# tonymisic/audio-visual-tubes

Hardware: AMD Instinct MI355X
Metric: train-step clips/sec (whole node), ResNet18+VGG-M hard-way loss at 1/2/4/8 GPU (higher is better)
Workload: dtype bf16; 1 GPU; train_hardway_1frame step: 224x224 RGB + 257x300 spectrogram, fwd+CE+bwd+Adam; configs[1]; global_batch=128, per_gpu_batch=128, parallelism=dp1

## Files before the change

audio-visual-tubes_amd/_lib.py:

```python
from __future__ import annotations

import ctypes
import os
import subprocess
import threading

PKG_DIR = os.path.dirname(os.path.abspath(__file__))
CSRC = os.path.join(PKG_DIR, "csrc")
LIB_PATH = os.path.join(PKG_DIR, "libavt.so")
LOAD_PATH = os.environ.get("AVT_LIB_PATH", LIB_PATH)
SOURCES = ["conv_gemm.hip", "bn.hip", "pool.hip", "head.hip", "misc.hip", "tube.hip", "conv3d_bwd.hip", "eval.hip", "audio.hip", "frames.hip"]

_P = ctypes.c_void_p
_I = ctypes.c_int
_L = ctypes.c_longlong
_F = ctypes.c_float
_Z = ctypes.c_size_t

class DgradBnEpi(ctypes.Structure):
    _fields_ = [("xc", ctypes.c_void_p), ("y", ctypes.c_void_p), ("stats", ctypes.c_void_p),
                ("acc", ctypes.c_void_p), ("xc2", ctypes.c_void_p), ("stats2", ctypes.c_void_p),
                ("acc2", ctypes.c_void_p), ("skip_class00", ctypes.c_int), ("append_slots", ctypes.c_int)]


# ... 27 lines not shown
    "avt_set_halo_stages": (_I, [_I, _I]),
    "avt_set_c64": (_I, [_I]),
    "avt_set_s2_dgrad_one": (_I, [_I]),
    "avt_set_stem_kernel": (_I, [_I]),
    "avt_set_stem_wgrad": (_I, [_I]),
    "avt_set_nt128_config": (_I, [_I]),
    "avt_set_wgrad_slab_max": (_I, [_I, _I]),
    "avt_set_wgrad_tiles": (_I, [_I]),
    "avt_set_small_tiles": (_I, [_I]),
    "avt_set_wgrad_halo": (_I, [_I]),
    "avt_set_wgrad_row3": (_I, [_I, _I, _I]),
    "avt_set_halo3d": (_I, [_I]),
    "avt_set_halo_tps2": (_I, [_I]),
    "avt_set_wgrad_fused": (_I, [_I, _I]),
    "avt_conv2d_wgrad_tickets": (_I, [_I, _I, _I, _I, _I, _I, _I, _I, _I, _I]),
    "avt_conv2d_wgrad_tk": (_I, [_P, _P, _P, _I, _I, _I, _I, _I, _I, _I, _I, _I, _I, _P, _Z, _P, _I, _P]),
    "avt_conv2d_wgrad_defer": (_I, [_P, _P, _P, _I, _I, _I, _I, _I, _I, _I, _I, _I, _I, _P, _Z,
                                    ctypes.POINTER(SlabReduceDesc), _P]),
    "avt_wgrad_reduce_batch": (_I, [ctypes.POINTER(SlabReduceDesc), _I, _P]),
    "avt_bn_acc_doubles": (_Z, [_L, _I]),
    "avt_conv2d_fwd": (_I, [_P, _P, _P, _P, _I, _I, _I, _I, _I, _I, _I, _I, _I, _I, _P]),
    "avt_conv2d_dgrad": (_I, [_P, _P, _P, _P, _I, _I, _I, _I, _I, _I, _I, _I, _I, _P]),
    "avt_conv2d_dgrad_bn": (_I, [_P, _P, _P, _P, _I, _I, _I, _I, _I, _I, _I, _I, _I, ctypes.POINTER(DgradBnEpi), _P]),
    "avt_bn_bwd_premasked": (_I, [_P, _P, _P, _P, _P, _P, _P, _P, _P, _L, _I, _P]),
    "avt_conv2d_dgrad_mask": (_I, [_P, _P, _P, _P, _P, _I, _I, _I, _I, _I, _I, _I, _I, _I, _P]),
    "avt_conv2d_splitk_plan": (_I, [_I, _I, _I, _I, _I, _I, _I, _I, _I, _I, _P, _P]),
    "avt_set_halo_splitk": (_I, [_I, _I]),
    "avt_set_wgrad_nst": (_I, [_I, _I]),
    "avt_set_wgrad_slots_pct": (_I, [_I]),
    "avt_conv2d_fwd_ws": (_I, [_P, _P, _P, _P, _I, _I, _I, _I, _I, _I, _I, _I, _I, _I, _P, _L, _P, _I, _P]),
    "avt_conv2d_dgrad_ws": (_I, [_P, _P, _P, _P, _P, _I, _I, _I, _I, _I, _I, _I, _I, _I, _P, _L, _P, _I, _P]),
    "avt_bn_apply_mask": (_I, [_P, _P, _P, _P, _P, _P, _P, _P, _L, _I, _P]),
    "avt_bn_bwd_mask": (_I, [_P, _P, ctypes.POINTER(BnBwdTarget), ctypes.POINTER(BnBwdTarget), _L, _I, _P]),
    "avt_conv2d_wgrad_workspace": (_Z, [_I, _I, _I, _I, _I, _I, _I, _I, _I, _I]),
    "avt_conv2d_wgrad": (_I, [_P, _P, _P, _I, _I, _I, _I, _I, _I, _I, _I, _I, _I, _P, _Z, _P]),
    "avt_bn_finalize": (_I, [_P, _L, _I, _P, _P, _P, _P, _F, _F, _P, _P, _P, _P, _P]),
    "avt_bn_finalize_rep": (_I, [_P, _L, _L, _I, _P, _P, _P, _P, _F, _F, _P, _P, _P, _P, _P]),
    "avt_conv3d_fwd": (_I, [_P, _P, _P, _P, _I, _I, _I, _I, _I, _I, _I, _I, _I, _I, _I, _I, _P]),
    "avt_video_stem_im2col": (_I, [_P, _P, _I, _I, _I, _I, _I, _I, _I, _P]),
    "avt_maxpool3d_fwd": (_I, [_P, _P, _I, _I, _I, _I, _I, _P]),
    "avt_pack_conv3d_weight_dgrad": (_I, [_P, _P, _I, _I, _I, _I, _I, _P]),
    "avt_pack_conv3d_weights_dgrad_batched": (_I, [_P, _I, _I, _P]),
    "avt_conv3d_dgrad": (_I, [_P, _P, _P, _P, _I, _I, _I, _I, _I, _I, _I, _I, _I, _I, _I, _I, _P]),
    "avt_conv3d_wgrad_workspace": (_Z, [_I, _I, _I, _I, _I, _I, _I, _I, _I, _I, _I, _I]),
    "avt_conv3d_wgrad": (_I, [_P, _P, _P, _I, _I, _I, _I, _I, _I, _I, _I, _I, _I, _I, _I, _P, _Z, _P]),
    "avt_maxpool3d_bwd": (_I, [_P, _P, _P, _P, _I, _I, _I, _I, _I, _P]),
# ... 152 lines not shown
```

audio-visual-tubes_amd/csrc/conv_epi.h:

```cpp
#pragma once

__device__ __forceinline__ u32x4 epi_mask8(u32x4 v, unsigned bits) {
  unsigned* u = reinterpret_cast<unsigned*>(&v);
#pragma unroll
  for (int e = 0; e < 4; ++e)
    u[e] &= ((bits >> (2 * e)) & 1u ? 0x0000ffffu : 0u) | ((bits >> (2 * e + 1)) & 1u ? 0xffff0000u : 0u);
  return v;
}

__device__ __forceinline__ void epi_unpack8(const u32x4& v, float* f) {
  const unsigned* u = reinterpret_cast<const unsigned*>(&v);
#pragma unroll
  for (int e = 0; e < 4; ++e) {
    f[2 * e] = bf2f(u[e] & 0xffff);
    f[2 * e + 1] = bf2f(u[e] >> 16);
  }
}

template <int NT, int BM, int BN, int UMAX, typename OrowFn>
__device__ __forceinline__ void epi_store_bn(const GemmNTParams& p, const bf16_t* Ct, int ct_ld, int n0, int rows_valid,
                                             int mt, int nrow_tiles, OrowFn orow, float* scratch) {
  constexpr int OCPR = BN / 8;
  static_assert(NT % OCPR == 0 && 64 % OCPR == 0, "a thread keeps one channel chunk");
  const int tid = threadIdx.x;
  const bool bnb = p.bx != nullptr;
  const bool two = p.bx2 != nullptr;
  const int cc = tid % OCPR;
  const int c0 = n0 + cc * 8;
  float s1[8], s2[8], s3[8];
#pragma unroll
  for (int e = 0; e < 8; ++e) s1[e] = s2[e] = s3[e] = 0.f;
  constexpr int ITERS = BM * OCPR / NT;
  static_assert(ITERS * NT == BM * OCPR, "rows per thread");
  constexpr int U = ITERS < UMAX ? ITERS : UMAX;
  const bool has_add = p.add != nullptr, has_y = p.by != nullptr;
  for (int it0 = 0; it0 < ITERS; it0 += U) {
    u32x4 aa[U], xx[U], yy[U], x2[U];
    size_t off[U];
// ... 45 lines not shown
          for (int e = 0; e < 8; ++e)
            g[e] = __builtin_fmaf(xc[e], bst[c0 + e], bst[p.Ng + c0 + e]) > 0.f ? g[e] : 0.f;
        }
#pragma unroll
        for (int e = 0; e < 8; ++e) {
          s1[e] += g[e];
          s2[e] += g[e] * ((xc[e] - bst[2 * p.Ng + c0 + e]) * bst[3 * p.Ng + c0 + e]);
        }
        if (two) {
          float xb[8];
          epi_unpack8(x2[u], xb);
#pragma unroll
          for (int e = 0; e < 8; ++e)
            s3[e] += g[e] * ((xb[e] - bst2[2 * p.Ng + c0 + e]) * bst2[3 * p.Ng + c0 + e]);
        }
        unsigned* vp = reinterpret_cast<unsigned*>(&v);
#pragma unroll
        for (int e = 0; e < 4; ++e) vp[e] = pack2(g[2 * e], g[2 * e + 1]);
      }
      *reinterpret_cast<u32x4*>(p.out + off[u]) = v;
    }
  }
  if (!bnb) return;
#pragma unroll
  for (int m = OCPR; m < 64; m <<= 1)
#pragma unroll
    for (int e = 0; e < 8; ++e) {
      s1[e] += __shfl_xor(s1[e], m, 64);
      s2[e] += __shfl_xor(s2[e], m, 64);
      if (two) s3[e] += __shfl_xor(s3[e], m, 64);
    }
  constexpr int NW = NT / 64;
  const int lane = tid & 63, wid = tid >> 6;
  __syncthreads();
  if (lane < OCPR) {
#pragma unroll
    for (int e = 0; e < 8; ++e) {
      float* q = scratch + ((size_t)wid * BN + cc * 8 + e) * 3;
      q[0] = s1[e];
      q[1] = s2[e];
      q[2] = s3[e];
    }
  }
  __syncthreads();
  const int total = p.bslot_total ? p.bslot_total : nrow_tiles;
  bn_write_header(p.bacc, total, p.bappend);
  if (two) bn_write_header(p.bacc2, total, p.bappend);
  const size_t slot = (size_t)(p.bslot_base + bn_slot_base(p.bacc, p.bappend) + mt);
  const size_t slot2 = two ? (size_t)(p.bslot_base + bn_slot_base(p.bacc2, p.bappend) + mt) : 0;
  for (int c = tid; c < BN; c += NT) {
    float a = 0.f, b = 0.f, d = 0.f;
#pragma unroll
    for (int w = 0; w < NW; ++w) {
      const float* q = scratch + ((size_t)w * BN + c) * 3;
      a += q[0];
      b += q[1];
      d += q[2];
    }
    double* acc = bn_bwd_slots(p.bacc, p.Ng) + (slot * p.Ng + n0 + c) * 2;
    acc[0] = (double)a;
    acc[1] = (double)b;
    if (two) {
      double* acc2 = bn_bwd_slots(p.bacc2, p.Ng) + (slot2 * p.Ng + n0 + c) * 2;
      acc2[0] = (double)a;
      acc2[1] = (double)d;
    }
  }
}

template <int NT, int BM, int BN, bool EPI, typename OrowFn, int UMAX = 4>
__device__ __forceinline__ void epi_store(const GemmNTParams& p, const bf16_t* Ct, int ct_ld, int n0, int rows_valid,
                                          int mt, int nrow_tiles, OrowFn orow, float* scratch) {
  if constexpr (!EPI) {
    constexpr int OCPR = BN / 8;
    for (int idx = threadIdx.x; idx < BM * OCPR; idx += NT) {
      const int r = idx / OCPR, cc = idx - r * OCPR;
      if (r >= rows_valid) continue;
      u32x4 v = *reinterpret_cast<const u32x4*>(Ct + r * ct_ld + cc * 8);
      const size_t off = orow(r) * (size_t)p.Ng + n0 + cc * 8;
      if (p.add != nullptr) {
        u32x4 a = *reinterpret_cast<const u32x4*>(p.add + off);
        if (p.amask != nullptr) a = epi_mask8(a, p.amask[off >> 3]);
        unsigned* vv = reinterpret_cast<unsigned*>(&v);
        const unsigned* aa = reinterpret_cast<const unsigned*>(&a);
#pragma unroll
        for (int e = 0; e < 4; ++e) {
          const float lo = bf2f(vv[e] & 0xffff) + bf2f(aa[e] & 0xffff);
          const float hi = bf2f(vv[e] >> 16) + bf2f(aa[e] >> 16);
          vv[e] = pack2(lo, hi);
        }
      }
      *reinterpret_cast<u32x4*>(p.out + off) = v;
    }
    return;
  } else {
    epi_store_bn<NT, BM, BN, UMAX>(p, Ct, ct_ld, n0, rows_valid, mt, nrow_tiles, orow, scratch);
  }
}
```

audio-visual-tubes_amd/csrc/conv_gemm.hip:

```cpp
#include "avt_common.h"

namespace avt {

#include "conv_params.h"

template <int MODE, int CVEC, int BM, int BN>
__global__ __launch_bounds__(256) void gemm_nt_kernel(GemmNTParams p) {
  constexpr int TM = BM / 64, TN = BN / 64;
  constexpr int AR = BM / 64, BR = BN / 64;
  constexpr int STAGE_BYTES = 2 * (BM + BN) * 64;
  constexpr int CT_LD = BN + 8;
  constexpr int EPI_BYTES = BM * CT_LD * 2;
  constexpr int SMEM = (STAGE_BYTES > EPI_BYTES ? STAGE_BYTES : EPI_BYTES);
  __shared__ __attribute__((aligned(16))) char smem[SMEM + 4 * BN * 4];
  float* red = reinterpret_cast<float*>(smem + SMEM);

  const int tid = threadIdx.x, lane = tid & 63, wid = tid >> 6;
  const int wm = wid >> 1, wn = wid & 1;
  const int nnt = p.Ng / BN;
  const int mt = blockIdx.x / nnt, nt = blockIdx.x % nnt;
  const int m0 = mt * BM, n0 = nt * BN;

  const int lchunk = tid & 3, lrow = tid >> 2;
  int a_pix[AR], a_y[AR], a_x[AR];
// ... 733 lines not shown
static bool halo_eligible(const GemmNTParams& p) {
  const int h = halo_enabled();
  if (!h || p.R != 3 || p.S != 3 || p.stride != 1 || p.pad != 1 || p.IC % 64 != 0 || p.IT > 1 || p.OT > 1 || p.KT > 1 ||
      p.IH != p.OH || p.IW != p.OW)
    return false;
  if (h == 2) return 256 + 2 * p.OW + 2 <= kHaloPR && (p.Ng % 128 == 0 || p.Ng == 64);
  static const int l2 = getenv("AVT_HALO_L2") ? atoi(getenv("AVT_HALO_L2")) : 1;
  return p.Ng % 128 == 0 && (128 + 2 * p.OW + 2 <= 168 || (l2 && 256 + 2 * p.OW + 2 <= kHaloPR));
}

static bool use_small_tile(const GemmNTParams& p, int BN) {
  if (g_small_tile_pct == -2) {
    const char* e = getenv("AVT_SMALL_TILES");
    const char* ep = getenv("AVT_SMALL_TILES_PCT");
    const int w = e ? atoi(e) : 1;
    g_small_tile_pct = e ? (w > 0 ? 100 * w : w) : ep ? atoi(ep) : 50;
  }
  if (g_small_tile_pct == 0) return false;
  if (g_small_tile_pct < 0) return true;
  const long long blocks128 = (long long)((p.M + 127) / 128) * (p.Ng / BN);
  return blocks128 * 100 < (long long)g_small_tile_pct * num_cus();
}

template <int MODE, int WM, int WN, int TM, int TN, int NSTB, int PRMAX, bool EPI, int OPT = 0>
static void launch_halo_one(const GemmNTParams& p, const HaloArgs& ha, int grid, hipStream_t st) {
  hipLaunchKernelGGL((conv_halo_kernel<MODE, WM, WN, TM, TN, NSTB, PRMAX, EPI, false, 0, OPT>), dim3(grid),
                     dim3(WM * WN * 64), 0, st, p, ha);
}

template <int MODE, int WM, int WN, int TM, int TN, int NSTB = 3, int PRMAX = kHaloPR, int OPT = 0>
static void launch_halo(const GemmNTParams& p, hipStream_t st, int ksplit = 1, float* part = nullptr,
                        int* cnt = nullptr) {
  constexpr int BM = WM * TM * 32, BN = WN * TN * 32;
  HaloArgs ha{};
  ha.ksplit = ksplit;
  ha.cps = p.IC / 64 / ksplit;
#ifdef AVT_DIAG
  static const int hdbg = getenv("AVT_HALO_DBG") ? atoi(getenv("AVT_HALO_DBG")) : 0;
  ha.dbg = hdbg;
#endif
  ha.part = part;
  ha.cnt = cnt;
  const int batch = p.M / (p.OH * p.OW);
  ha.act_bytes = (unsigned)((size_t)batch * p.IH * p.IW * p.IC * 2);
  ha.w_bytes = (unsigned)((size_t)p.Ng * p.Kg * 2);
  ha.W = p.OW;
  ha.H = p.OH;
  for (int r = 0; r < 3; ++r)
    for (int s = 0; s < 3; ++s) {
      const int t = r * 3 + s;
      const int dy = MODE == MODE_FWD ? r - 1 : 1 - r, dx = MODE == MODE_FWD ? s - 1 : 1 - s;
      ha.tap_dy[t] = dy;
      ha.tap_dx[t] = dx;
      ha.tap_disp[t] = dy * p.OW + dx;
      ha.tap_w[t] = t;
    }
  if constexpr ((OPT & 4) != 0) {
    ha.T = p.IT;
    ha.div_hw = make_magic((unsigned)(p.OH * p.OW));
    ha.div_t = make_magic((unsigned)p.IT);
  }
  const int grid = ((p.M + BM - 1) / BM) * (p.Ng / BN) * ksplit;
  if (grid > 0 && ksplit > 1) {
    hipLaunchKernelGGL((conv_halo_kernel<MODE, WM, WN, TM, TN, NSTB, PRMAX, false, true>), dim3(grid),
                       dim3(WM * WN * 64), 0, st, p, ha);
    return;
  }
  if (grid <= 0) return;
  if constexpr ((OPT & 4) != 0)
    launch_halo_one<MODE, WM, WN, TM, TN, NSTB, PRMAX, false, OPT>(p, ha, grid, st);
  else if (MODE == MODE_DGRAD && p.bx != nullptr)
    launch_halo_one<MODE, WM, WN, TM, TN, NSTB, PRMAX, true, OPT>(p, ha, grid, st);
  else
    launch_halo_one<MODE, WM, WN, TM, TN, NSTB, PRMAX, false, OPT>(p, ha, grid, st);
}

static int g_halo_tps2 = -1;
static int halo_tps2(const GemmNTParams& p, int vt = 1) {
  if (g_halo_tps2 < 0) g_halo_tps2 = getenv("AVT_HALO_TPS2") ? atoi(getenv("AVT_HALO_TPS2")) : 0;
  const int nv = p.IC / 64 * vt;
  return g_halo_tps2 && p.IC % 64 == 0 && nv % 2 == 0 && nv >= 8;
}

static int g_halo3d = -1;
static int halo3d_enabled() {
  if (g_halo3d < 0) g_halo3d = getenv("AVT_HALO3D") ? atoi(getenv("AVT_HALO3D")) : 2;
  return g_halo3d;
}
static bool halo3d_launch(const GemmNTParams& p, hipStream_t st) {
  if (!halo3d_enabled() || p.KT != 3 || p.R != 3 || p.S != 3 || p.stride != 1 || p.pad != 1 || p.pad_t != 1 ||
      p.IT != p.OT || p.IH != p.OH || p.IW != p.OW || p.IC % 64 != 0 || conv_variant() != 1)
    return false;
  if (p.Ng == 64) {
    if (halo3d_enabled() < 2 || 256 + 2 * p.OW + 2 > 488) return false;
    launch_halo<MODE_FWD, 8, 1, 1, 2, 3, 488, 4>(p, st);
    return true;
  }
// ... 364 lines not shown
  if (C % 128 == 0)
    launch_nt<MODE_DGRAD, 8, 128, 128>(p, st, ws);
  else
    launch_nt<MODE_DGRAD, 8, 128, 64>(p, st);
  return check_launch("conv2d_dgrad");
}

extern "C" int avt_conv2d_dgrad_ws(const void* dy, const void* wt, void* dx, const void* add, const void* add_mask,
                                   int N, int H, int W, int C, int K, int R, int S, int stride, int pad, float* part,
                                   long long part_floats, int* cnt, int counters, void* stream) {
  AVT_REQUIRE(add_mask == nullptr || (add && add != dx), "conv2d_dgrad_ws: add_mask needs add, not aliasing dx");
  AVT_REQUIRE(part_floats >= 0 && counters >= 0, "conv2d_dgrad_ws: negative workspace size");
  const SplitWs ws{part, cnt, part_floats, counters};
  return conv2d_dgrad_impl(dy, wt, dx, add, add_mask, N, H, W, C, K, R, S, stride, pad, nullptr, stream,
                           (part && cnt) ? &ws : nullptr);
}

extern "C" int avt_conv2d_dgrad_bn(const void* dy, const void* wt, void* dx, const void* add, int N, int H, int W,
                                   int C, int K, int R, int S, int stride, int pad, const avt_dgrad_bn_epi* epi,
                                   void* stream) {
  return conv2d_dgrad_impl(dy, wt, dx, add, nullptr, N, H, W, C, K, R, S, stride, pad, epi, stream);
}

extern "C" int avt_conv2d_dgrad(const void* dy, const void* wt, void* dx, const void* add, int N, int H, int W, int C,
                                int K, int R, int S, int stride, int pad, void* stream) {
  return conv2d_dgrad_impl(dy, wt, dx, add, nullptr, N, H, W, C, K, R, S, stride, pad, nullptr, stream);
}

extern "C" int avt_conv2d_dgrad_mask(const void* dy, const void* wt, void* dx, const void* add, const void* add_mask,
                                     int N, int H, int W, int C, int K, int R, int S, int stride, int pad,
                                     void* stream) {
  AVT_REQUIRE(add && add_mask, "conv2d_dgrad_mask: add and add_mask are required");
  AVT_REQUIRE(add != dx, "conv2d_dgrad_mask: add must not alias dx");
  return conv2d_dgrad_impl(dy, wt, dx, add, add_mask, N, H, W, C, K, R, S, stride, pad, nullptr, stream);
}

static int conv3d_fwd_impl(const void* x, const void* wpack, void* y, double* bn_acc, const void* add, int N, int T,
                           int H, int W, int Cp, int K, int KT, int R, int S, int stride, int pad_t, int pad,
                           void* stream) {
  AVT_REQUIRE(x && wpack && y, "conv3d_fwd: null pointer");
  AVT_REQUIRE(K % 64 == 0, "conv3d_fwd: K=%d must be a multiple of 64", K);
  AVT_REQUIRE(Cp % 32 == 0, "conv3d_fwd: C=%d must be a multiple of 32", Cp);
  AVT_REQUIRE(KT * R * S <= kMaxTaps && KT >= 1 && R >= 1 && S >= 1, "conv3d_fwd: at most %d taps", kMaxTaps);
  AVT_REQUIRE(stride == 1 || stride == 2, "conv3d_fwd: spatial stride must be 1 or 2");
  GemmNTParams p{};
  p.act = (const bf16_t*)x;
// ... 692 lines not shown
```

audio-visual-tubes_amd/csrc/conv_halo.h:

```cpp
#pragma once

struct HaloArgs {
  unsigned act_bytes, w_bytes;
  int W, H;
  int tap_disp[9];
  int tap_dy[9], tap_dx[9];
  int tap_w[9];
  int ksplit, cps;
  float* part;
  int* cnt;
  int dbg;
  int T;
  MagicDiv div_hw, div_t;
};
#ifdef AVT_DIAG
#define HALO_DBG(bit) (ha.dbg & (bit))
#else
#define HALO_DBG(bit) false
#endif


__device__ __forceinline__ int halo_swz(int row) { return (row >> 1) & 7; }

template <int WN, int TN, int NSTB, int PRMAX, int TPS = 1>
constexpr int halo_blocks_per_cu() {
  return 2 * (2 * (PRMAX * 128 + 1024) + NSTB * TPS * WN * TN * 32 * 128 + 4096) <= 160 * 1024 ? 2 : 1;
}

template <int MODE, int WM, int WN, int TM, int TN, int NSTB, int PRMAX, bool EPI = false, bool SPLIT = false,
          int PREF = 0, int OPT = 0>
__global__ __launch_bounds__(WM * WN * 64, (halo_blocks_per_cu<WN, TN, NSTB, PRMAX, (OPT & 2) ? 2 : 1>())) void conv_halo_kernel(
    GemmNTParams p, HaloArgs ha) {
  constexpr int FR = 32, FM = TM, FN = TN;
  constexpr int KD = 16;
  constexpr int NW = WM * WN, NT = NW * 64;
  constexpr int BM = WM * TM * 32, BN = WN * TN * 32;
  constexpr int BK = 64, RB = 128, RPI = 8;
  constexpr int BR = BN / (NW * RPI);
  static_assert(BR >= 1 && BR * NW * RPI == BN, "weight tile / wave split");
  constexpr int PINSTR = (PRMAX + RPI - 1) / RPI;
  static_assert(NSTB >= 2 && NSTB <= 5, "NSTB");
  constexpr int NPIECE = 10 - NSTB;
  constexpr int AP = (PINSTR + NPIECE * NW - 1) / (NPIECE * NW);
  constexpr int ABUF = PRMAX * RB + 1024;
  constexpr int BSTAGE = BN * RB;
  constexpr int TPS = (OPT & 2) ? 2 : 1;
  constexpr int CT_LD = BN + 8;
  constexpr int EPI_BYTES = BM * CT_LD * 2;
  constexpr int MAIN = 2 * ABUF + NSTB * TPS * BSTAGE;
  constexpr int SMEM = (MAIN > EPI_BYTES ? MAIN : EPI_BYTES);
  static_assert(PRMAX % RPI == 0, "PRMAX");
  static_assert(SMEM + 2 * WM * BN * 4 <= 160 * 1024, "LDS budget of a CU");
// ... 411 lines not shown
          if (acc_row(i, v) < rows_valid) q += d * d;
        }
#pragma unroll
      for (int o = FR; o < 64; o <<= 1) q += __shfl_xor(q, o, 64);
      if (lane < FR) red[WM * BN + wm * BN + cc] = q;
    }
    __syncthreads();
    bn_write_header(p.stats, (p.M + BM - 1) / BM, 0, mt == 0 && n0 == 0);
    double* acc_slot = bn_fwd_slots(p.stats) + (size_t)mt * p.Ng * 3;
    for (int cc = tid; cc < BN; cc += NT) {
      double sd = 0.0, m2 = 0.0;
#pragma unroll
      for (int k = 0; k < WM; ++k) {
        sd += (double)red[k * BN + cc];
        m2 += (double)red[WM * BN + k * BN + cc];
      }
      double* a = acc_slot + (size_t)(n0 + cc) * 3;
      a[0] = sd;
      a[1] = m2;
      a[2] = sd * sd / (double)rows_valid;
    }
  }
  bf16_t* Ct = reinterpret_cast<bf16_t*>(smem);
#pragma unroll
  for (int i = 0; i < FM; ++i)
#pragma unroll
    for (int j = 0; j < FN; ++j)
#pragma unroll
      for (int v = 0; v < AV; ++v) Ct[acc_row(i, v) * CT_LD + wn * (BN / WN) + j * FR + frow] = f2bf(acc[i][j][v]);
  __syncthreads();
  if (!HALO_DBG(16))
    epi_store<NT, BM, BN, EPI>(p, Ct, CT_LD, n0, rows_valid, mt, (p.M + BM - 1) / BM,
                               [&](int r) -> size_t { return (size_t)(m0 + r); },
                        reinterpret_cast<float*>(smem));
}
```

audio-visual-tubes_amd/trunk.py:

```python
from __future__ import annotations

import ctypes
import os
from dataclasses import dataclass
from typing import Dict, List, Optional

import torch

from ._lib import BnBwdTarget, DgradBnEpi, SlabReduceDesc, call, query

STAGES = [(64, 1), (128, 2), (256, 2), (512, 1)]
FUSE_BN_BWD = os.environ.get("AVT_FUSE_BN_BWD", "0") == "1"
DIAG_H1_SKIP = os.environ.get("AVT_DIAG_H1_SKIP", "0") == "1"
if DIAG_H1_SKIP and os.environ.get("AVT_DIAG_WRONG_RESULTS_OK", "0") != "1":
    raise RuntimeError("avt: AVT_DIAG_H1_SKIP=1 computes WRONG results (timing diagnostic); set "
                       "AVT_DIAG_WRONG_RESULTS_OK=1 as well to run it (tools/step_time.py)")


def P(t: Optional[torch.Tensor]):
    return None if t is None else ctypes.c_void_p(t.data_ptr())


def stream_ptr():
    return ctypes.c_void_p(torch.cuda.current_stream().cuda_stream)


def drive(gen):
    while True:
        try:
            next(gen)
        except StopIteration as e:
            return e.value


def conv_out(n: int, k: int, s: int, p: int) -> int:
# ... 304 lines not shown
                pending.append((d, ws))
        else:
            call("avt_conv2d_wgrad_tk", P(x), P(gy), P(dw), N, H, W, spec.cp, spec.cin, spec.cout, spec.k, spec.k,
                 spec.stride, spec.pad, P(ws), wsb, P(tk), 0 if tk is None else tk.numel(), stream_ptr())
        ConvProfiler.end(ev, "wgrad", 2.0 * gy.numel() * spec.k * spec.k * spec.cin,
                         2.0 * (x.numel() + gy.numel()) + 8.0 * dw.numel())

    def flush_wgrad(self, store: Store):
        pending = store.wgrad_pending(self.prefix)
        if not pending:
            return
        arr = (SlabReduceDesc * len(pending))(*[d for d, _ in pending])
        call("avt_wgrad_reduce_batch", arr, len(pending), stream_ptr())
        pending.clear()

    def _dgrad(self, gy, N, H, W, spec: ConvSpec, store: Store, add=None, inplace=False, epi=None, add_mask=None):
        _, wt = store.packed(spec)
        gx = add if inplace else torch.empty(N, H, W, spec.cin, device=gy.device, dtype=torch.bfloat16)
        ws = store.splitk(spec, True, N, H, W) if epi is None else None
        ev = ConvProfiler.begin()
        if ws is not None:
            call("avt_conv2d_dgrad_ws", P(gy), P(wt), P(gx), P(add), P(add_mask), N, H, W, spec.cin, spec.cout,
                 spec.k, spec.k, spec.stride, spec.pad, P(ws[0]), ws[0].numel(), P(ws[1]), ws[1].numel(), stream_ptr())
        elif add_mask is not None:
            assert epi is None
            call("avt_conv2d_dgrad_mask", P(gy), P(wt), P(gx), P(add), P(add_mask), N, H, W, spec.cin, spec.cout,
                 spec.k, spec.k, spec.stride, spec.pad, stream_ptr())
        elif epi is None:
            call("avt_conv2d_dgrad", P(gy), P(wt), P(gx), P(add), N, H, W, spec.cin, spec.cout, spec.k, spec.k,
                 spec.stride, spec.pad, stream_ptr())
        else:
            call("avt_conv2d_dgrad_bn", P(gy), P(wt), P(gx), P(add), N, H, W, spec.cin, spec.cout, spec.k, spec.k,
                 spec.stride, spec.pad, ctypes.byref(epi), stream_ptr())
        ConvProfiler.end(ev, "dgrad", 2.0 * gy.numel() * spec.k * spec.k * spec.cin,
                         2.0 * (gy.numel() + wt.numel() + gx.numel() * (2 if add is not None else 1)))
        return gx

    HI_BLOCK = 4

    def backward(self, tape: Dict, g_out: torch.Tensor, store: Store, on_boundary=None):
        g, pm = self.backward_blocks(tape, g_out, store, self.HI_BLOCK, len(self.blocks))
        if on_boundary is not None:
            on_boundary(self.prefix + "hi")
        g, _ = self.backward_blocks(tape, g, store, 0, self.HI_BLOCK, pm)
        self.backward_stem(tape, g, store)

    def _bn_bwd_premasked(self, gm, xc, stats, bn: BNSpec, store: Store):
        gc = torch.empty_like(xc)
        call("avt_bn_bwd_premasked", P(gm), P(xc), P(stats[2]), P(stats[3]), P(store.param(bn.prefix + ".weight")),
             P(store.grad(bn.prefix + ".weight")), P(store.grad(bn.prefix + ".bias")), P(gc),
             P(store.stat_acc(bn, "bwd", xc.numel() // bn.c)), xc.numel() // bn.c, bn.c, stream_ptr())
        return gc

    def _epi(self, store: Store, bn: BNSpec, xc, stats, y=None, bn2: Optional[BNSpec] = None, xc2=None, stats2=None,
             skip00: bool = False, append: bool = False) -> DgradBnEpi:
        e = DgradBnEpi()
        rows = xc.numel() // bn.c
        e.xc, e.y, e.stats = xc.data_ptr(), (y.data_ptr() if y is not None else None), stats.data_ptr()
        e.acc = store.stat_acc(bn, "bwd", rows).data_ptr()
        if bn2 is not None:
            e.xc2, e.stats2, e.acc2 = xc2.data_ptr(), stats2.data_ptr(), store.stat_acc(bn2, "bwd", rows).data_ptr()
        e.skip_class00 = int(skip00)
        e.append_slots = int(append)
        return e

    def backward_blocks(self, tape: Dict, g: torch.Tensor, store: Store, lo: int, hi: int, premasked: bool = False):
        return drive(self.backward_blocks_iter(tape, g, store, lo, hi, premasked))

    def backward_blocks_iter(self, tape: Dict, g: torch.Tensor, store: Store, lo: int, hi: int,
                             premasked: bool = False):
        N = tape["N"]
        ev = not tape.get("training", True)
        pgrad = not (ev and tape.get("frozen", False))
        fuse = FUSE_BN_BWD and not ev
        for bi in reversed(range(lo, hi)):
            blk, t = self.blocks[bi], tape["blocks"][bi]
            Hc, Wc, Ho, Wo = t["H"], t["W"], t["Ho"], t["Wo"]
            identity = blk["down"] is None
            if premasked:
                gres = g
                g_c2 = self._bn_bwd_premasked(g, t["c2"], t["s2"], blk["bn2"], store)
                g_cd = None if identity else self._bn_bwd_premasked(g, t["cd"], t["sd"], blk["bnd"], store)
            else:
                gres = None
                if ev:
                    g_c2, g_cd = self._bn_eval_bwd_mask(g, t["om"], t["c2"], t["s2"], blk["bn2"], store, pgrad,
                                                        *(() if identity else (t["cd"], t["sd"], blk["bnd"])))
                elif identity and fuse and bi > 0:
                    gres = torch.empty_like(t["c2"])
                    g_c2 = self._bn_bwd(g, t["out"], t["c2"], t["s2"], blk["bn2"], store, gmask_out=gres)
                    g_cd = None
                elif identity:
                    g_c2, g_cd = self._bn_bwd_mask(g, t["om"], t["c2"], t["s2"], blk["bn2"], store)
                else:
                    g_c2, g_cd = self._bn_bwd_mask(g, t["om"], t["c2"], t["s2"], blk["bn2"], store,
                                                   t["cd"], t["sd"], blk["bnd"])
            yield
            if pgrad:
                self._wgrad(t["h1"], g_c2, N, Ho, Wo, blk["conv2"], store)
            yield
            if fuse:
                g_h1 = self._dgrad(g_c2, N, Ho, Wo, blk["conv2"], store,
                                   epi=self._epi(store, blk["bn1"], t["c1"], t["s1"]))
                g_c1 = self._bn_bwd_premasked(g_h1, t["c1"], t["s1"], blk["bn1"], store)
            else:
                g_h1 = self._dgrad(g_c2, N, Ho, Wo, blk["conv2"], store)
                yield
                if ev:
                    g_c1 = self._bn_eval_relu_bwd(g_h1, t["c1"], t["s1"], blk["bn1"], store, pgrad)
                else:
                    g_c1 = self._bn_relu_bwd(g_h1, t["c1"], t["s1"], blk["bn1"], store)
            yield
            if pgrad:
                self._wgrad(t["x"], g_c1, N, Hc, Wc, blk["conv1"], store)
                yield
                if not identity:
                    self._wgrad(t["x"], g_cd, N, Hc, Wc, blk["down"], store)
                    yield
            epi = None
            if bi > 0 and fuse:
                pb, pt = self.blocks[bi - 1], tape["blocks"][bi - 1]
                has_d = pb["down"] is not None
                mk = lambda skip00, append=False: self._epi(
                    store, pb["bn2"], pt["c2"], pt["s2"], y=pt["out"], bn2=pb["bnd"] if has_d else None,
                    xc2=pt["cd"] if has_d else None, stats2=pt["sd"] if has_d else None, skip00=skip00, append=append)
                epi = mk(False)
            if identity and gres is None:
                g_x = self._dgrad(g_c1, N, Hc, Wc, blk["conv1"], store, add=g, epi=epi, add_mask=t["om"])
            elif identity:
                g_x = self._dgrad(g_c1, N, Hc, Wc, blk["conv1"], store, add=gres, epi=epi)
            else:
                strided = blk["conv1"].stride == 2
                g_x = self._dgrad(g_c1, N, Hc, Wc, blk["conv1"], store,
                                  epi=mk(True) if (epi is not None and strided) else None)
                if epi is not None and strided:
                    epi = mk(False, append=True)
                g_x = self._dgrad(g_cd, N, Hc, Wc, blk["down"], store, add=g_x, inplace=True, epi=epi)
            g = g_x
            premasked = epi is not None
            yield
        return g, premasked

    def backward_stem(self, tape: Dict, g: torch.Tensor, store: Store):
# ... 38 lines not shown
```

include/avt.h:

```cpp
#ifndef AVT_H_
#define AVT_H_

#include <stddef.h>

#ifdef __cplusplus
extern "C" {
#endif

#define AVT_OK 0
#define AVT_EINVAL -1
#define AVT_EHIP -2

const char* avt_last_error(void);
int avt_abi_version(void);
#define AVT_BUILD_DIAG 1
int avt_build_flags(void);

int avt_peak_mfma(float* sink, int shape, int blocks, int iters, unsigned seed, void* stream);
long long avt_peak_mfma_flops(int shape, int blocks, int iters);
int avt_copy16(void* dst, const void* src, size_t bytes, int blocks, void* stream);

size_t avt_bn_acc_doubles(long long rows, int C);
int avt_conv2d_fwd(const void* x, const void* wpack, void* y, double* bn_acc, int N, int H, int W, int Cp, int K,
                   int R, int S, int stride, int pad, int Kg, void* stream);
// ... 2 lines not shown
int avt_conv2d_dgrad_mask(const void* dy, const void* wt, void* dx, const void* add, const void* add_mask, int N,
                          int H, int W, int C, int K, int R, int S, int stride, int pad, void* stream);
int avt_conv2d_splitk_plan(int N, int H, int W, int C, int K, int R, int S, int stride, int pad, int dgrad,
                           long long* part_floats, int* counters);
int avt_conv2d_fwd_ws(const void* x, const void* wpack, void* y, double* bn_acc, int N, int H, int W, int Cp, int K,
                      int R, int S, int stride, int pad, int Kg, float* part, long long part_floats, int* cnt,
                      int counters, void* stream);
int avt_conv2d_dgrad_ws(const void* dy, const void* wt, void* dx, const void* add, const void* add_mask, int N,
                        int H, int W, int C, int K, int R, int S, int stride, int pad, float* part,
                        long long part_floats, int* cnt, int counters, void* stream);
typedef struct {
  const void* xc;
  const void* y;
  const float* stats;
  double* acc;
  const void* xc2;
  const float* stats2;
  double* acc2;
  int skip_class00;
  int append_slots;
} avt_dgrad_bn_epi;
int avt_conv2d_dgrad_bn(const void* dy, const void* wt, void* dx, const void* add, int N, int H, int W, int C, int K,
                        int R, int S, int stride, int pad, const avt_dgrad_bn_epi* epi, void* stream);
size_t avt_conv2d_wgrad_workspace(int N, int H, int W, int Cp, int Creal, int K, int R, int S, int stride, int pad);
int avt_conv2d_wgrad(const void* x, const void* dy, float* dw, int N, int H, int W, int Cp, int Creal, int K, int R,
                     int S, int stride, int pad, void* workspace, size_t ws_bytes, void* stream);
typedef struct {
  const float* slab;
  float* dw;
  int splits, tiles, nnt, Mg, ldw;
  int wm, wn, tm, tn;
} avt_slab_reduce_desc;
int avt_conv2d_wgrad_defer(const void* x, const void* dy, float* dw, int N, int H, int W, int Cp, int Creal, int K,
                           int R, int S, int stride, int pad, void* workspace, size_t ws_bytes, avt_slab_reduce_desc* desc,
                           void* stream);
int avt_wgrad_reduce_batch(const avt_slab_reduce_desc* descs, int n, void* stream);
int avt_conv2d_wgrad_tickets(int N, int H, int W, int Cp, int Creal, int K, int R, int S, int stride, int pad);
int avt_conv2d_wgrad_tk(const void* x, const void* dy, float* dw, int N, int H, int W, int Cp, int Creal, int K, int R,
                        int S, int stride, int pad, void* workspace, size_t ws_bytes, int* tickets, int n_tickets,
                        void* stream);

int avt_conv_stem_dgrad(const void* gy, const float* w, float* gx, int N, int H, int W, int Cin, void* stream);

int avt_conv3d_fwd(const void* x, const void* wpack, void* y, double* bn_acc, int N, int T, int H, int W, int Cp,
                   int K, int KT, int R, int S, int stride, int pad_t, int pad, void* stream);
int avt_video_stem_im2col(const float* x, void* out, int N, int C, int T, int H, int W, int KT, int pad_t,
// ... 140 lines not shown
```

Before: 13060 clips/s.

## Enable fused BN-backward dgrad epilogue by default with per-shape planning

Turns BN-backward fusion into the dgrad halo kernel on by default, but only for conv2 shapes where a planner confirms the halo path is used without split-K. Adds a restructured halo epilogue that prefetches the BN inputs and per-channel constants into registers and LDS before the accumulator store, plus a specialised variant without residual or mask operands. Also adds a masked-add dgrad+BN entry point. This removes separate BN-backward reduction passes and their memory traffic, at the cost of more register and LDS pressure in the epilogue, and relies on the planner's heuristic choice of shapes.

```diff
diff --git a/audio-visual-tubes_amd/_lib.py b/audio-visual-tubes_amd/_lib.py
--- a/audio-visual-tubes_amd/_lib.py
+++ b/audio-visual-tubes_amd/_lib.py
@@ -73,6 +73,9 @@
     "avt_conv2d_fwd": (_I, [_P, _P, _P, _P, _I, _I, _I, _I, _I, _I, _I, _I, _I, _I, _P]),
     "avt_conv2d_dgrad": (_I, [_P, _P, _P, _P, _I, _I, _I, _I, _I, _I, _I, _I, _I, _P]),
     "avt_conv2d_dgrad_bn": (_I, [_P, _P, _P, _P, _I, _I, _I, _I, _I, _I, _I, _I, _I, ctypes.POINTER(DgradBnEpi), _P]),
+    "avt_conv2d_dgrad_bn_mask": (_I, [_P, _P, _P, _P, _P, _I, _I, _I, _I, _I, _I, _I, _I, _I,
+                                      ctypes.POINTER(DgradBnEpi), _P]),
+    "avt_conv2d_dgrad_bn_plan": (_I, [_I, _I, _I, _I, _I, _I, _I, _I, _I, _P]),
     "avt_bn_bwd_premasked": (_I, [_P, _P, _P, _P, _P, _P, _P, _P, _P, _L, _I, _P]),
     "avt_conv2d_dgrad_mask": (_I, [_P, _P, _P, _P, _P, _I, _I, _I, _I, _I, _I, _I, _I, _I, _P]),
     "avt_conv2d_splitk_plan": (_I, [_I, _I, _I, _I, _I, _I, _I, _I, _I, _I, _P, _P]),
diff --git a/audio-visual-tubes_amd/csrc/conv_epi.h b/audio-visual-tubes_amd/csrc/conv_epi.h
--- a/audio-visual-tubes_amd/csrc/conv_epi.h
+++ b/audio-visual-tubes_amd/csrc/conv_epi.h
@@ -14,6 +14,59 @@
   for (int e = 0; e < 4; ++e) {
     f[2 * e] = bf2f(u[e] & 0xffff);
     f[2 * e + 1] = bf2f(u[e] >> 16);
+  }
+}
+
+template <int NT, int BN>
+__device__ __forceinline__ void epi_bn_tail(const GemmNTParams& p, float* s1, float* s2, float* s3, int n0, int mt,
+                                            int nrow_tiles, float* scratch) {
+  constexpr int OCPR = BN / 8;
+  const int tid = threadIdx.x;
+  const bool two = p.bx2 != nullptr;
+  const int cc = tid % OCPR;
+#pragma unroll
+  for (int m = OCPR; m < 64; m <<= 1)
+#pragma unroll
+    for (int e = 0; e < 8; ++e) {
+      s1[e] += __shfl_xor(s1[e], m, 64);
+      s2[e] += __shfl_xor(s2[e], m, 64);
+      if (two) s3[e] += __shfl_xor(s3[e], m, 64);
+    }
+  constexpr int NW = NT / 64;
+  const int lane = tid & 63, wid = tid >> 6;
+  __syncthreads();
+  if (lane < OCPR) {
+#pragma unroll
+    for (int e = 0; e < 8; ++e) {
+      float* q = scratch + ((size_t)wid * BN + cc * 8 + e) * 3;
+      q[0] = s1[e];
+      q[1] = s2[e];
+      q[2] = s3[e];
+    }
+  }
+  __syncthreads();
+  const int total = p.bslot_total ? p.bslot_total : nrow_tiles;
+  bn_write_header(p.bacc, total, p.bappend);
+  if (two) bn_write_header(p.bacc2, total, p.bappend);
+  const size_t slot = (size_t)(p.bslot_base + bn_slot_base(p.bacc, p.bappend) + mt);
+  const size_t slot2 = two ? (size_t)(p.bslot_base + bn_slot_base(p.bacc2, p.bappend) + mt) : 0;
+  for (int c = tid; c < BN; c += NT) {
+    float a = 0.f, b = 0.f, d = 0.f;
+#pragma unroll
+    for (int w = 0; w < NW; ++w) {
+      const float* q = scratch + ((size_t)w * BN + c) * 3;
+      a += q[0];
+      b += q[1];
+      d += q[2];
+    }
+    double* acc = bn_bwd_slots(p.bacc, p.Ng) + (slot * p.Ng + n0 + c) * 2;
+    acc[0] = (double)a;
+    acc[1] = (double)b;
+    if (two) {
+      double* acc2 = bn_bwd_slots(p.bacc2, p.Ng) + (slot2 * p.Ng + n0 + c) * 2;
+      acc2[0] = (double)a;
+      acc2[1] = (double)d;
+    }
   }
 }
 
@@ -105,50 +158,7 @@
     }
   }
   if (!bnb) return;
-#pragma unroll
-  for (int m = OCPR; m < 64; m <<= 1)
-#pragma unroll
-    for (int e = 0; e < 8; ++e) {
-      s1[e] += __shfl_xor(s1[e], m, 64);
-      s2[e] += __shfl_xor(s2[e], m, 64);
-      if (two) s3[e] += __shfl_xor(s3[e], m, 64);
-    }
-  constexpr int NW = NT / 64;
-  const int lane = tid & 63, wid = tid >> 6;
-  __syncthreads();
-  if (lane < OCPR) {
-#pragma unroll
-    for (int e = 0; e < 8; ++e) {
-      float* q = scratch + ((size_t)wid * BN + cc * 8 + e) * 3;
-      q[0] = s1[e];
-      q[1] = s2[e];
-      q[2] = s3[e];
-    }
-  }
-  __syncthreads();
-  const int total = p.bslot_total ? p.bslot_total : nrow_tiles;
-  bn_write_header(p.bacc, total, p.bappend);
-  if (two) bn_write_header(p.bacc2, total, p.bappend);
-  const size_t slot = (size_t)(p.bslot_base + bn_slot_base(p.bacc, p.bappend) + mt);
-  const size_t slot2 = two ? (size_t)(p.bslot_base + bn_slot_base(p.bacc2, p.bappend) + mt) : 0;
-  for (int c = tid; c < BN; c += NT) {
-    float a = 0.f, b = 0.f, d = 0.f;
-#pragma unroll
-    for (int w = 0; w < NW; ++w) {
-      const float* q = scratch + ((size_t)w * BN + c) * 3;
-      a += q[0];
-      b += q[1];
-      d += q[2];
-    }
-    double* acc = bn_bwd_slots(p.bacc, p.Ng) + (slot * p.Ng + n0 + c) * 2;
-    acc[0] = (double)a;
-    acc[1] = (double)b;
-    if (two) {
-      double* acc2 = bn_bwd_slots(p.bacc2, p.Ng) + (slot2 * p.Ng + n0 + c) * 2;
-      acc2[0] = (double)a;
-      acc2[1] = (double)d;
-    }
-  }
+  epi_bn_tail<NT, BN>(p, s1, s2, s3, n0, mt, nrow_tiles, scratch);
 }
 
 template <int NT, int BM, int BN, bool EPI, typename OrowFn, int UMAX = 4>
@@ -180,3 +190,115 @@
     epi_store_bn<NT, BM, BN, UMAX>(p, Ct, ct_ld, n0, rows_valid, mt, nrow_tiles, orow, scratch);
   }
 }
+
+template <int NT, int BM, int BN, bool GEN>
+struct EpiBnHalo {
+  static constexpr int OCPR = BN / 8;
+  static constexpr int ITERS = BM * OCPR / NT;
+  static constexpr int CST_FLOATS = 6 * BN;
+  static_assert(NT % OCPR == 0 && 64 % OCPR == 0 && ITERS * NT == BM * OCPR && NT >= BN, "rows per thread");
+  u32x4 xx[ITERS];
+  u32x4 aa[GEN ? ITERS : 1], yy[GEN ? ITERS : 1], x2[GEN ? ITERS : 1];
+  unsigned am[GEN ? ITERS : 1];
+  float kc[6];
+
+  __device__ __forceinline__ void load(const GemmNTParams& p, int n0, size_t m0, int rows_valid) {
+    const int tid = threadIdx.x;
+    const int c0 = n0 + (tid % OCPR) * 8;
+    if (tid < BN) {
+#pragma unroll
+      for (int k = 0; k < 4; ++k) kc[k] = p.bst[k * p.Ng + n0 + tid];
+      if (GEN && p.bx2 != nullptr) {
+        kc[4] = p.bst2[2 * p.Ng + n0 + tid];
+        kc[5] = p.bst2[3 * p.Ng + n0 + tid];
+      }
+    }
+#pragma unroll
+    for (int u = 0; u < ITERS; ++u) {
+      const int r = (tid + u * NT) / OCPR;
+      if (r >= rows_valid) continue;
+      const size_t off = (m0 + r) * (size_t)p.Ng + c0;
+      xx[u] = *reinterpret_cast<const u32x4*>(p.bx + off);
+      if constexpr (GEN) {
+        if (p.by != nullptr) yy[u] = *reinterpret_cast<const u32x4*>(p.by + off);
+        if (p.bx2 != nullptr) x2[u] = *reinterpret_cast<const u32x4*>(p.bx2 + off);
+        if (p.add != nullptr) {
+          aa[u] = *reinterpret_cast<const u32x4*>(p.add + off);
+          if (p.amask != nullptr) am[u] = p.amask[off >> 3];
+        }
+      }
+    }
+  }
+
+  __device__ __forceinline__ void stage_consts(const GemmNTParams& p, float* cst) const {
+    const int tid = threadIdx.x;
+    if (tid < BN) {
+#pragma unroll
+      for (int k = 0; k < 4; ++k) cst[k * BN + tid] = kc[k];
+      if (GEN && p.bx2 != nullptr) {
+        cst[4 * BN + tid] = kc[4];
+        cst[5 * BN + tid] = kc[5];
+      }
+    }
+  }
+
+  __device__ __forceinline__ void finish(const GemmNTParams& p, const bf16_t* Ct, int ct_ld, int n0, size_t m0,
+                                         int rows_valid, int mt, int nrow_tiles, const float* cst, float* scratch) {
+    const int tid = threadIdx.x;
+    const int cc = tid % OCPR;
+    const int c0 = n0 + cc * 8;
+    const bool two = GEN && p.bx2 != nullptr, has_y = GEN && p.by != nullptr, has_add = GEN && p.add != nullptr;
+    const bool has_am = has_add && p.amask != nullptr;
+    const float* kq = cst + cc * 8;
+    float s1[8], s2[8], s3[8];
+#pragma unroll
+    for (int e = 0; e < 8; ++e) s1[e] = s2[e] = s3[e] = 0.f;
+#pragma unroll
+    for (int u = 0; u < ITERS; ++u) {
+      const int r = (tid + u * NT) / OCPR;
+      if (r >= rows_valid) continue;
+      u32x4 v = *reinterpret_cast<const u32x4*>(Ct + r * ct_ld + cc * 8);
+      if constexpr (GEN) {
+        if (has_add) {
+          const u32x4 a = has_am ? epi_mask8(aa[u], am[u]) : aa[u];
+          unsigned* vp = reinterpret_cast<unsigned*>(&v);
+          const unsigned* ap = reinterpret_cast<const unsigned*>(&a);
+#pragma unroll
+          for (int e = 0; e < 4; ++e) {
+            const float lo = bf2f(vp[e] & 0xffff) + bf2f(ap[e] & 0xffff);
+            const float hi = bf2f(vp[e] >> 16) + bf2f(ap[e] >> 16);
+            vp[e] = pack2(lo, hi);
+          }
+        }
+      }
+      float g[8], xc[8];
+      epi_unpack8(v, g);
+      epi_unpack8(xx[u], xc);
+      if (has_y) {
+        float y[8];
+        epi_unpack8(yy[GEN ? u : 0], y);
+#pragma unroll
+        for (int e = 0; e < 8; ++e) g[e] = y[e] > 0.f ? g[e] : 0.f;
+      } else {
+#pragma unroll
+        for (int e = 0; e < 8; ++e) g[e] = __builtin_fmaf(xc[e], kq[e], kq[BN + e]) > 0.f ? g[e] : 0.f;
+      }
+#pragma unroll
+      for (int e = 0; e < 8; ++e) {
+        s1[e] += g[e];
+        s2[e] += g[e] * ((xc[e] - kq[2 * BN + e]) * kq[3 * BN + e]);
+      }
+      if (two) {
+        float xb[8];
+        epi_unpack8(x2[GEN ? u : 0], xb);
+#pragma unroll
+        for (int e = 0; e < 8; ++e) s3[e] += g[e] * ((xb[e] - kq[4 * BN + e]) * kq[5 * BN + e]);
+      }
+      unsigned* vp = reinterpret_cast<unsigned*>(&v);
+#pragma unroll
+      for (int e = 0; e < 4; ++e) vp[e] = pack2(g[2 * e], g[2 * e + 1]);
+      *reinterpret_cast<u32x4*>(p.out + ((m0 + r) * (size_t)p.Ng + c0)) = v;
+    }
+    epi_bn_tail<NT, BN>(p, s1, s2, s3, n0, mt, nrow_tiles, scratch);
+  }
+};
diff --git a/audio-visual-tubes_amd/csrc/conv_gemm.hip b/audio-visual-tubes_amd/csrc/conv_gemm.hip
--- a/audio-visual-tubes_amd/csrc/conv_gemm.hip
+++ b/audio-visual-tubes_amd/csrc/conv_gemm.hip
@@ -779,7 +779,7 @@
   return blocks128 * 100 < (long long)g_small_tile_pct * num_cus();
 }
 
-template <int MODE, int WM, int WN, int TM, int TN, int NSTB, int PRMAX, bool EPI, int OPT = 0>
+template <int MODE, int WM, int WN, int TM, int TN, int NSTB, int PRMAX, int EPI, int OPT = 0>
 static void launch_halo_one(const GemmNTParams& p, const HaloArgs& ha, int grid, hipStream_t st) {
   hipLaunchKernelGGL((conv_halo_kernel<MODE, WM, WN, TM, TN, NSTB, PRMAX, EPI, false, 0, OPT>), dim3(grid),
                      dim3(WM * WN * 64), 0, st, p, ha);
@@ -819,17 +819,22 @@
   }
   const int grid = ((p.M + BM - 1) / BM) * (p.Ng / BN) * ksplit;
   if (grid > 0 && ksplit > 1) {
-    hipLaunchKernelGGL((conv_halo_kernel<MODE, WM, WN, TM, TN, NSTB, PRMAX, false, true>), dim3(grid),
+    hipLaunchKernelGGL((conv_halo_kernel<MODE, WM, WN, TM, TN, NSTB, PRMAX, 0, true>), dim3(grid),
                        dim3(WM * WN * 64), 0, st, p, ha);
     return;
   }
   if (grid <= 0) return;
   if constexpr ((OPT & 4) != 0)
-    launch_halo_one<MODE, WM, WN, TM, TN, NSTB, PRMAX, false, OPT>(p, ha, grid, st);
-  else if (MODE == MODE_DGRAD && p.bx != nullptr)
-    launch_halo_one<MODE, WM, WN, TM, TN, NSTB, PRMAX, true, OPT>(p, ha, grid, st);
-  else
-    launch_halo_one<MODE, WM, WN, TM, TN, NSTB, PRMAX, false, OPT>(p, ha, grid, st);
+    launch_halo_one<MODE, WM, WN, TM, TN, NSTB, PRMAX, 0, OPT>(p, ha, grid, st);
+  else if (MODE == MODE_DGRAD && p.bx != nullptr) {
+    if constexpr (MODE == MODE_DGRAD) {
+      if (p.by == nullptr && p.bx2 == nullptr && p.add == nullptr)
+        launch_halo_one<MODE, WM, WN, TM, TN, NSTB, PRMAX, 1, OPT>(p, ha, grid, st);
+      else
+        launch_halo_one<MODE, WM, WN, TM, TN, NSTB, PRMAX, 2, OPT>(p, ha, grid, st);
+    }
+  } else
+    launch_halo_one<MODE, WM, WN, TM, TN, NSTB, PRMAX, 0, OPT>(p, ha, grid, st);
 }
 
 static int g_halo_tps2 = -1;
@@ -1240,6 +1245,35 @@
   return conv2d_dgrad_impl(dy, wt, dx, add, nullptr, N, H, W, C, K, R, S, stride, pad, epi, stream);
 }
 
+extern "C" int avt_conv2d_dgrad_bn_mask(const void* dy, const void* wt, void* dx, const void* add,
+                                        const void* add_mask, int N, int H, int W, int C, int K, int R, int S,
+                                        int stride, int pad, const avt_dgrad_bn_epi* epi, void* stream) {
+  AVT_REQUIRE(add && add_mask && epi, "conv2d_dgrad_bn_mask: add, add_mask and epi are required");
+  AVT_REQUIRE(add != dx, "conv2d_dgrad_bn_mask: add must not alias dx");
+  return conv2d_dgrad_impl(dy, wt, dx, add, add_mask, N, H, W, C, K, R, S, stride, pad, epi, stream);
+}
+
+extern "C" int avt_conv2d_dgrad_bn_plan(int N, int H, int W, int C, int K, int R, int S, int stride, int pad,
+                                        int* fuse) {
+  AVT_REQUIRE(fuse, "conv2d_dgrad_bn_plan: null pointer");
+  *fuse = 0;
+  if (C % 64 != 0 || K % 32 != 0 || (stride != 1 && stride != 2) || N <= 0) return AVT_OK;
+  GemmNTParams p{};
+  p.IH = conv_out(H, R, stride, pad);
+  p.IW = conv_out(W, S, stride, pad);
+  p.IC = K;
+  p.OH = H; p.OW = W;
+  p.IT = p.OT = p.KT = 1;
+  p.M = N * H * W;
+  p.Ng = C;
+  p.Kg = R * S * K;
+  p.R = R; p.S = S; p.stride = stride; p.pad = pad;
+  if (p.M <= 0 || C % 128 != 0 || conv_variant() != 1 || !halo_eligible(p)) return AVT_OK;
+  if (g_nt128_config < 0 && (g_nt64_config < 0 || g_nt64_config == 1) && use_small_tile(p, 128)) return AVT_OK;
+  *fuse = 1;
+  return AVT_OK;
+}
+
 extern "C" int avt_conv2d_dgrad(const void* dy, const void* wt, void* dx, const void* add, int N, int H, int W, int C,
                                 int K, int R, int S, int stride, int pad, void* stream) {
   return conv2d_dgrad_impl(dy, wt, dx, add, nullptr, N, H, W, C, K, R, S, stride, pad, nullptr, stream);
diff --git a/audio-visual-tubes_amd/csrc/conv_halo.h b/audio-visual-tubes_amd/csrc/conv_halo.h
--- a/audio-visual-tubes_amd/csrc/conv_halo.h
+++ b/audio-visual-tubes_amd/csrc/conv_halo.h
@@ -27,7 +27,7 @@
   return 2 * (2 * (PRMAX * 128 + 1024) + NSTB * TPS * WN * TN * 32 * 128 + 4096) <= 160 * 1024 ? 2 : 1;
 }
 
-template <int MODE, int WM, int WN, int TM, int TN, int NSTB, int PRMAX, bool EPI = false, bool SPLIT = false,
+template <int MODE, int WM, int WN, int TM, int TN, int NSTB, int PRMAX, int EPI = 0, bool SPLIT = false,
           int PREF = 0, int OPT = 0>
 __global__ __launch_bounds__(WM * WN * 64, (halo_blocks_per_cu<WN, TN, NSTB, PRMAX, (OPT & 2) ? 2 : 1>())) void conv_halo_kernel(
     GemmNTParams p, HaloArgs ha) {
@@ -485,15 +485,26 @@
     }
   }
   bf16_t* Ct = reinterpret_cast<bf16_t*>(smem);
+  constexpr int CST_OFF = (EPI_BYTES + 15) & ~15;
+  static_assert(!EPI || (MODE == MODE_DGRAD && !SPLIT), "BN-backward epilogue: a dgrad, no split-K");
+  static_assert(!EPI || CST_OFF + 6 * BN * 4 <= SMEM, "the epilogue's constants fit in the main loop's LDS");
+  static_assert(!EPI || NW * BN * 3 * 4 <= EPI_BYTES, "the epilogue's cross-wave scratch stays inside Ct");
+  float* cst = reinterpret_cast<float*>(smem + CST_OFF);
+  EpiBnHalo<NT, BM, BN, EPI == 2> ebn;
+  if constexpr (EPI != 0) ebn.load(p, n0, (size_t)m0, rows_valid);
 #pragma unroll
   for (int i = 0; i < FM; ++i)
 #pragma unroll
     for (int j = 0; j < FN; ++j)
 #pragma unroll
       for (int v = 0; v < AV; ++v) Ct[acc_row(i, v) * CT_LD + wn * (BN / WN) + j * FR + frow] = f2bf(acc[i][j][v]);
+  if constexpr (EPI != 0) ebn.stage_consts(p, cst);
   __syncthreads();
-  if (!HALO_DBG(16))
-    epi_store<NT, BM, BN, EPI>(p, Ct, CT_LD, n0, rows_valid, mt, (p.M + BM - 1) / BM,
-                               [&](int r) -> size_t { return (size_t)(m0 + r); },
-                        reinterpret_cast<float*>(smem));
+  if constexpr (EPI != 0) {
+    ebn.finish(p, Ct, CT_LD, n0, (size_t)m0, rows_valid, mt, (p.M + BM - 1) / BM, cst, reinterpret_cast<float*>(smem));
+  } else {
+    if (!HALO_DBG(16))
+      epi_store<NT, BM, BN, false>(p, Ct, CT_LD, n0, rows_valid, mt, (p.M + BM - 1) / BM,
+                                   [&](int r) -> size_t { return (size_t)(m0 + r); }, reinterpret_cast<float*>(smem));
+  }
 }
diff --git a/audio-visual-tubes_amd/trunk.py b/audio-visual-tubes_amd/trunk.py
--- a/audio-visual-tubes_amd/trunk.py
+++ b/audio-visual-tubes_amd/trunk.py
@@ -10,7 +10,8 @@
 from ._lib import BnBwdTarget, DgradBnEpi, SlabReduceDesc, call, query
 
 STAGES = [(64, 1), (128, 2), (256, 2), (512, 1)]
-FUSE_BN_BWD = os.environ.get("AVT_FUSE_BN_BWD", "0") == "1"
+FUSE_BN_BWD = os.environ.get("AVT_FUSE_BN_BWD", "") != "0"
+FUSE_BN_BWD_ALL = os.environ.get("AVT_FUSE_BN_BWD", "") == "1"
 DIAG_H1_SKIP = os.environ.get("AVT_DIAG_H1_SKIP", "0") == "1"
 if DIAG_H1_SKIP and os.environ.get("AVT_DIAG_WRONG_RESULTS_OK", "0") != "1":
     raise RuntimeError("avt: AVT_DIAG_H1_SKIP=1 computes WRONG results (timing diagnostic); set "
@@ -361,10 +362,12 @@
         if ws is not None:
             call("avt_conv2d_dgrad_ws", P(gy), P(wt), P(gx), P(add), P(add_mask), N, H, W, spec.cin, spec.cout,
                  spec.k, spec.k, spec.stride, spec.pad, P(ws[0]), ws[0].numel(), P(ws[1]), ws[1].numel(), stream_ptr())
-        elif add_mask is not None:
-            assert epi is None
+        elif add_mask is not None and epi is None:
             call("avt_conv2d_dgrad_mask", P(gy), P(wt), P(gx), P(add), P(add_mask), N, H, W, spec.cin, spec.cout,
                  spec.k, spec.k, spec.stride, spec.pad, stream_ptr())
+        elif add_mask is not None:
+            call("avt_conv2d_dgrad_bn_mask", P(gy), P(wt), P(gx), P(add), P(add_mask), N, H, W, spec.cin, spec.cout,
+                 spec.k, spec.k, spec.stride, spec.pad, ctypes.byref(epi), stream_ptr())
         elif epi is None:
             call("avt_conv2d_dgrad", P(gy), P(wt), P(gx), P(add), N, H, W, spec.cin, spec.cout, spec.k, spec.k,
                  spec.stride, spec.pad, stream_ptr())
@@ -403,6 +406,19 @@
         e.append_slots = int(append)
         return e
 
+    @staticmethod
+    def _fuses(spec: ConvSpec, N, H, W, store: Store) -> bool:
+        if not FUSE_BN_BWD:
+            return False
+        if FUSE_BN_BWD_ALL:
+            return True
+        if store.splitk(spec, True, N, H, W) is not None:
+            return False
+        f = ctypes.c_int(0)
+        call("avt_conv2d_dgrad_bn_plan", N, H, W, spec.cin, spec.cout, spec.k, spec.k, spec.stride, spec.pad,
+             ctypes.byref(f))
+        return bool(f.value)
+
     def backward_blocks(self, tape: Dict, g: torch.Tensor, store: Store, lo: int, hi: int, premasked: bool = False):
         return drive(self.backward_blocks_iter(tape, g, store, lo, hi, premasked))
 
@@ -416,6 +432,8 @@
             blk, t = self.blocks[bi], tape["blocks"][bi]
             Hc, Wc, Ho, Wo = t["H"], t["W"], t["Ho"], t["Wo"]
             identity = blk["down"] is None
+            fuse2 = fuse and self._fuses(blk["conv2"], N, Ho, Wo, store)
+            fuse1 = fuse and bi > 0 and FUSE_BN_BWD_ALL
             if premasked:
                 gres = g
                 g_c2 = self._bn_bwd_premasked(g, t["c2"], t["s2"], blk["bn2"], store)
@@ -425,7 +443,7 @@
                 if ev:
                     g_c2, g_cd = self._bn_eval_bwd_mask(g, t["om"], t["c2"], t["s2"], blk["bn2"], store, pgrad,
                                                         *(() if identity else (t["cd"], t["sd"], blk["bnd"])))
-                elif identity and fuse and bi > 0:
+                elif identity and fuse1 and FUSE_BN_BWD_ALL:
                     gres = torch.empty_like(t["c2"])
                     g_c2 = self._bn_bwd(g, t["out"], t["c2"], t["s2"], blk["bn2"], store, gmask_out=gres)
                     g_cd = None
@@ -438,7 +456,7 @@
             if pgrad:
                 self._wgrad(t["h1"], g_c2, N, Ho, Wo, blk["conv2"], store)
             yield
-            if fuse:
+            if fuse2:
                 g_h1 = self._dgrad(g_c2, N, Ho, Wo, blk["conv2"], store,
                                    epi=self._epi(store, blk["bn1"], t["c1"], t["s1"]))
                 g_c1 = self._bn_bwd_premasked(g_h1, t["c1"], t["s1"], blk["bn1"], store)
@@ -457,7 +475,7 @@
                     self._wgrad(t["x"], g_cd, N, Hc, Wc, blk["down"], store)
                     yield
             epi = None
-            if bi > 0 and fuse:
+            if fuse1:
                 pb, pt = self.blocks[bi - 1], tape["blocks"][bi - 1]
                 has_d = pb["down"] is not None
                 mk = lambda skip00, append=False: self._epi(
diff --git a/include/avt.h b/include/avt.h
--- a/include/avt.h
+++ b/include/avt.h
@@ -48,6 +48,10 @@
 } avt_dgrad_bn_epi;
 int avt_conv2d_dgrad_bn(const void* dy, const void* wt, void* dx, const void* add, int N, int H, int W, int C, int K,
                         int R, int S, int stride, int pad, const avt_dgrad_bn_epi* epi, void* stream);
+int avt_conv2d_dgrad_bn_mask(const void* dy, const void* wt, void* dx, const void* add, const void* add_mask, int N,
+                             int H, int W, int C, int K, int R, int S, int stride, int pad,
+                             const avt_dgrad_bn_epi* epi, void* stream);
+int avt_conv2d_dgrad_bn_plan(int N, int H, int W, int C, int K, int R, int S, int stride, int pad, int* fuse);
 size_t avt_conv2d_wgrad_workspace(int N, int H, int W, int Cp, int Creal, int K, int R, int S, int stride, int pad);
 int avt_conv2d_wgrad(const void* x, const void* dy, float* dw, int N, int H, int W, int Cp, int Creal, int K, int R,
                      int S, int stride, int pad, void* workspace, size_t ws_bytes, void* stream);
```

Result: no change. 13120 clips/s (median of 6 runs) (+0.5%).
